# Veason-silverbullet/NNR

Hardware: NVIDIA B200
Metric: cne_sue_train_impressions_per_sec (higher is better)
Workload: dtype f32

## Files before the change

nnr_b200/csrc/gemm_tc.cu:

```cuda
#include "common.cuh"
#include "gemm_epilogue.cuh"
#include <cuda.h>
#include <cuda_bf16.h>
#include <stdlib.h>

extern "C" int nnr_gemm_default_algo(void);

#define TC_BM 128
#define TC_THREADS 320
#define TC_TMEM_COLS 512
#define TC_ACC_COLS 256
#define TC_EPI_PITCH 80
#define TC_EPI_SCRATCH (8 * 32 * TC_EPI_PITCH)
#define TC_SMEM_BUDGET (205 * 1024)
#define TC_CHAIN_K 2048

__device__ __forceinline__ uint32_t smem_u32(const void* p) { return (uint32_t)__cvta_generic_to_shared(p); }

__device__ __forceinline__ void mbar_init(uint64_t* bar, uint32_t count) {
  asm volatile("mbarrier.init.shared::cta.b64 [%0], %1;" ::"r"(smem_u32(bar)), "r"(count));
}
__device__ __forceinline__ void mbar_expect_tx(uint64_t* bar, uint32_t bytes) {
  asm volatile("mbarrier.arrive.expect_tx.shared::cta.b64 _, [%0], %1;" ::"r"(smem_u32(bar)), "r"(bytes) : "memory");
}
// ... 16 lines not shown
__device__ __forceinline__ void tma_load_3d(const CUtensorMap* map, uint64_t* bar, uint32_t dst, int c0, int c1, int c2) {
  asm volatile(
      "cp.async.bulk.tensor.3d.shared::cluster.global.mbarrier::complete_tx::bytes [%0], [%1, {%3, %4, %5}], [%2];"
      ::"r"(dst), "l"(map), "r"(smem_u32(bar)), "r"(c0), "r"(c1), "r"(c2)
      : "memory");
}
__device__ __forceinline__ void tc_fence_before() { asm volatile("tcgen05.fence::before_thread_sync;" ::: "memory"); }
__device__ __forceinline__ void tc_fence_after() { asm volatile("tcgen05.fence::after_thread_sync;" ::: "memory"); }
__device__ __forceinline__ void tc_commit(uint64_t* bar) {
  asm volatile("tcgen05.commit.cta_group::1.mbarrier::arrive::one.shared::cluster.b64 [%0];" ::"r"(smem_u32(bar)) : "memory");
}
template <bool BF16>
__device__ __forceinline__ void tc_mma(uint32_t d_tmem, uint64_t a_desc, uint64_t b_desc, uint32_t idesc, uint32_t accumulate) {
  if (BF16) {
    asm volatile(
        "{\n.reg .pred p;\nsetp.ne.b32 p, %4, 0;\n"
        "tcgen05.mma.cta_group::1.kind::f16 [%0], %1, %2, %3, p;\n}\n" ::"r"(d_tmem), "l"(a_desc), "l"(b_desc), "r"(idesc),
        "r"(accumulate)
        : "memory");
  } else {
    asm volatile(
        "{\n.reg .pred p;\nsetp.ne.b32 p, %4, 0;\n"
        "tcgen05.mma.cta_group::1.kind::tf32 [%0], %1, %2, %3, p;\n}\n" ::"r"(d_tmem), "l"(a_desc), "l"(b_desc), "r"(idesc),
        "r"(accumulate)
        : "memory");
  }
}
__device__ __forceinline__ uint32_t cluster_ctarank() {
  uint32_t r;
  asm volatile("mov.u32 %0, %%cluster_ctarank;" : "=r"(r));
  return r;
}
__device__ __forceinline__ uint32_t mapa_rank(uint32_t addr, uint32_t rank) {
  uint32_t r;
  asm volatile("mapa.shared::cluster.u32 %0, %1, %2;" : "=r"(r) : "r"(addr), "r"(rank));
  return r;
}
__device__ __forceinline__ void cluster_sync_all() {
  asm volatile("barrier.cluster.arrive.release.aligned;\nbarrier.cluster.wait.acquire.aligned;" ::: "memory");
}
__device__ __forceinline__ void tma_load_3d_pair(const CUtensorMap* map, uint32_t leader_bar, uint32_t dst, int c0, int c1, int c2) {
  asm volatile(
      "cp.async.bulk.tensor.3d.cta_group::2.shared::cluster.global.mbarrier::complete_tx::bytes [%0], [%1, {%3, %4, %5}], [%2];"
      ::"r"(dst), "l"(map), "r"(leader_bar), "r"(c0), "r"(c1), "r"(c2)
      : "memory");
}
__device__ __forceinline__ void tc_commit_pair(uint64_t* bar) {
  asm volatile("tcgen05.commit.cta_group::2.mbarrier::arrive::one.shared::cluster.multicast::cluster.b64 [%0], %1;" ::"r"(smem_u32(bar)),
               "h"((uint16_t)3)
               : "memory");
}
__device__ __forceinline__ void mbar_arrive_cluster(uint32_t cluster_addr) {
  asm volatile("mbarrier.arrive.release.cluster.shared::cluster.b64 _, [%0];" ::"r"(cluster_addr) : "memory");
}
template <bool BF16>
__device__ __forceinline__ void tc_mma_pair(uint32_t d_tmem, uint64_t a_desc, uint64_t b_desc, uint32_t idesc, uint32_t accumulate) {
  if (BF16) {
    asm volatile(
        "{\n.reg .pred p;\nsetp.ne.b32 p, %4, 0;\n"
        "tcgen05.mma.cta_group::2.kind::f16 [%0], %1, %2, %3, p;\n}\n" ::"r"(d_tmem), "l"(a_desc), "l"(b_desc), "r"(idesc),
        "r"(accumulate)
        : "memory");
  } else {
    asm volatile(
        "{\n.reg .pred p;\nsetp.ne.b32 p, %4, 0;\n"
        "tcgen05.mma.cta_group::2.kind::tf32 [%0], %1, %2, %3, p;\n}\n" ::"r"(d_tmem), "l"(a_desc), "l"(b_desc), "r"(idesc),
        "r"(accumulate)
        : "memory");
  }
}

__device__ __forceinline__ void tmem_ld16(uint32_t taddr, float* v) {
  uint32_t r[16];
  asm volatile(
      "tcgen05.ld.sync.aligned.32x32b.x16.b32 {%0, %1, %2, %3, %4, %5, %6, %7, %8, %9, %10, %11, %12, %13, %14, %15}, [%16];"
      : "=r"(r[0]), "=r"(r[1]), "=r"(r[2]), "=r"(r[3]), "=r"(r[4]), "=r"(r[5]), "=r"(r[6]), "=r"(r[7]), "=r"(r[8]), "=r"(r[9]),
        "=r"(r[10]), "=r"(r[11]), "=r"(r[12]), "=r"(r[13]), "=r"(r[14]), "=r"(r[15])
      : "r"(taddr));
  asm volatile("tcgen05.wait::ld.sync.aligned;" ::: "memory");
#pragma unroll
  for (int i = 0; i < 16; ++i) v[i] = __uint_as_float(r[i]);
}

__device__ __forceinline__ uint64_t make_sw128_desc(uint32_t smem_addr, uint32_t lbo_bytes, uint32_t sbo_bytes, uint32_t layout_type) {
  uint64_t d = 0;
  d |= (uint64_t)((smem_addr & 0x3FFFF) >> 4);
  d |= (uint64_t)((lbo_bytes >> 4) & 0x3FFF) << 16;
  d |= (uint64_t)((sbo_bytes >> 4) & 0x3FFF) << 32;
  d |= (uint64_t)1 << 46;
  d |= (uint64_t)layout_type << 61;
  return d;
}

#ifdef NNR_TC_PROF
__device__ unsigned long long g_tc_prof[16];
#define TC_STAMP(i) { if (blockIdx.x == 0) g_tc_prof[i] = clock64(); }
#else
#define TC_STAMP(i) {}
#endif

struct TcParams {
  int M, N, K;
  const int32_t* m_dev;
  const int32_t* k_dev;
  int block_n, stages, nplanes;
  int a_mn, b_mn;
// ... 178 lines not shown
            v.x *= ks[0]; v.y *= ks[1]; v.z *= ks[2]; v.w *= ks[3];
          }
        } else if (EP == NNR_EPI_GATE) {
          v.x = sigmoid_fast(v.x + rb[i].x); v.y = sigmoid_fast(v.y + rb[i].y);
          v.z = sigmoid_fast(v.z + rb[i].z); v.w = sigmoid_fast(v.w + rb[i].w);
          if (p.epi.aux_out) *reinterpret_cast<float4*>(p.epi.aux_out + t.o_ao[i] + n) = v;
          v.x *= ax[i].x; v.y *= ax[i].y; v.z *= ax[i].z; v.w *= ax[i].w;
        } else if (EP == NNR_EPI_ADD_AUX) {
          v.x += ax[i].x; v.y += ax[i].y; v.z += ax[i].z; v.w += ax[i].w;
        }
        if (acc_early) { v.x += ax[i].x; v.y += ax[i].y; v.z += ax[i].z; v.w += ax[i].w; }
        else if (accumulate) {
          const float4 cc = *reinterpret_cast<const float4*>(Cout + t.o_c[i] + n);
          v.x += cc.x; v.y += cc.y; v.z += cc.z; v.w += cc.w;
        }
        *reinterpret_cast<float4*>(Cout + t.o_c[i] + n) = v;
        if (planes) {
          const __nv_bfloat162 h01 = __floats2bfloat162_rn(v.x, v.y), h23 = __floats2bfloat162_rn(v.z, v.w);
          __nv_bfloat16* op = p.c_planes + (long long)(t.row0 + 8 * i) * p.c_pitch + n;
          uint2 hv;
          hv.x = *reinterpret_cast<const uint32_t*>(&h01); hv.y = *reinterpret_cast<const uint32_t*>(&h23);
          *reinterpret_cast<uint2*>(op) = hv;
          if (p.c_lo) {
            const __nv_bfloat162 l01 = __floats2bfloat162_rn(v.x - __low2float(h01), v.y - __high2float(h01));
            const __nv_bfloat162 l23 = __floats2bfloat162_rn(v.z - __low2float(h23), v.w - __high2float(h23));
            uint2 lv;
            lv.x = *reinterpret_cast<const uint32_t*>(&l01); lv.y = *reinterpret_cast<const uint32_t*>(&l23);
            *reinterpret_cast<uint2*>(op + p.c_pstride) = lv;
          }
        }
      }
      if (planes) {
        const int mz = min(p.c_rows, (M + 63) & ~63);
#pragma unroll
        for (int i = 0; i < 4; ++i) {
          const int mm = t.row0 + 8 * i;
          if (mm >= M && mm < mz) {
            __nv_bfloat16* op = p.c_planes + (long long)mm * p.c_pitch + n;
            *reinterpret_cast<uint2*>(op) = make_uint2(0u, 0u);
            if (p.c_lo) *reinterpret_cast<uint2*>(op + p.c_pstride) = make_uint2(0u, 0u);
          }
        }
      }
    }
    __syncwarp();
    if (AHEAD && more) {
      bb = bbn;
#pragma unroll
      for (int i = 0; i < 4; ++i) { ax[i] = axn[i]; rb[i] = rbn[i]; }
    }
  }
}

template <bool BF16, bool PAIR, int EPK>
__global__ void __launch_bounds__(TC_THREADS, 1) gemm_tc_kernel(const __grid_constant__ CUtensorMap map_a,
                                                                const __grid_constant__ CUtensorMap map_b, TcParams p) {
  extern __shared__ __align__(1024) unsigned char smem_raw[];
  constexpr int KELEM = BF16 ? 64 : 32;
  constexpr int TILE_M = PAIR ? 2 * TC_BM : TC_BM;
  int M = p.M, K = p.K;
  if (p.m_dev) M = min(M, *p.m_dev);
  if (p.k_dev) K = min(K, *p.k_dev);
  const int warp = threadIdx.x >> 5, lane = threadIdx.x & 31;
  if (threadIdx.x == 0) TC_STAMP(0)
  const uint32_t rank = PAIR ? cluster_ctarank() : 0u;
  const int sched_id = PAIR ? (int)(blockIdx.x >> 1) : (int)blockIdx.x;
  const int sched_n = PAIR ? (int)(gridDim.x >> 1) : (int)gridDim.x;
  const int b_rows = PAIR ? (p.block_n >> 1) : p.block_n;

  const int m_tiles = (M + TILE_M - 1) / TILE_M;
  const int n_tiles = (p.N + p.block_n - 1) / p.block_n;
  const int nkb = (K + KELEM - 1) / KELEM;
  const int kb_per = p.split_k ? p.chain_kb : max(nkb, 1);
  const int splits = p.split_k ? max(1, (nkb + kb_per - 1) / kb_per) : 1;
  const int total_tiles = m_tiles * n_tiles * splits;

  const uint32_t a_tile = TC_BM * 128, b_tile = (uint32_t)b_rows * 128;
  const uint32_t stage_bytes = (uint32_t)p.nplanes * (a_tile + b_tile);
  unsigned char* tiles = (unsigned char*)(((uintptr_t)smem_raw + 1023) & ~(uintptr_t)1023);
  unsigned char* epi_scratch = tiles + (size_t)p.stages * stage_bytes;
  uint64_t* full_bar = reinterpret_cast<uint64_t*>(epi_scratch + TC_EPI_SCRATCH);
  uint64_t* empty_bar = full_bar + p.stages;
  uint64_t* tmem_full = empty_bar + p.stages;
  uint64_t* tmem_empty = tmem_full + 2;
  uint32_t* tmem_slot = reinterpret_cast<uint32_t*>(tmem_empty + 2);

  if (warp == 0 && lane == 0) {
    asm volatile("prefetch.tensormap [%0];" ::"l"(&map_a) : "memory");
    asm volatile("prefetch.tensormap [%0];" ::"l"(&map_b) : "memory");
    for (int s = 0; s < p.stages; ++s) { mbar_init(&full_bar[s], 1); mbar_init(&empty_bar[s], 1); }
    for (int b = 0; b < 2; ++b) { mbar_init(&tmem_full[b], 1); mbar_init(&tmem_empty[b], PAIR ? 16 : 8); }
    asm volatile("fence.mbarrier_init.release.cluster;" ::: "memory");
  }
  if (PAIR) cluster_sync_all();
  if (warp == 1) {
    if (PAIR) {
      asm volatile("tcgen05.alloc.cta_group::2.sync.aligned.shared::cta.b32 [%0], %1;" ::"r"(smem_u32(tmem_slot)), "n"(TC_TMEM_COLS) : "memory");
      asm volatile("tcgen05.relinquish_alloc_permit.cta_group::2.sync.aligned;" ::: "memory");
    } else {
      asm volatile("tcgen05.alloc.cta_group::1.sync.aligned.shared::cta.b32 [%0], %1;" ::"r"(smem_u32(tmem_slot)), "n"(TC_TMEM_COLS) : "memory");
      asm volatile("tcgen05.relinquish_alloc_permit.cta_group::1.sync.aligned;" ::: "memory");
    }
  }
  tc_fence_before();
  __syncthreads();
  tc_fence_after();
  const uint32_t tmem_base = *tmem_slot;
  if (threadIdx.x == 0) TC_STAMP(1)

  if (warp == 0) {
    if (lane == 0) {
      int it = 0;
      for (int tile = sched_id; tile < total_tiles; tile += sched_n) {
        const int n_idx = tile % n_tiles, rest = tile / n_tiles;
        const int m0 = (rest % m_tiles) * TILE_M + (int)rank * TC_BM, n0 = n_idx * p.block_n + (int)rank * b_rows, z = rest / m_tiles;
        const int kb0 = z * kb_per, kb1 = min(nkb, kb0 + kb_per);
        for (int kb = kb0; kb < kb1; ++kb, ++it) {
          const int s = it % p.stages;
          const uint32_t ph = (it / p.stages) & 1;
          mbar_wait(&empty_bar[s], ph ^ 1);
          const uint32_t base = smem_u32(tiles + (size_t)s * stage_bytes);
          if (!PAIR) mbar_expect_tx(&full_bar[s], stage_bytes);
          else if (rank == 0) mbar_expect_tx(&full_bar[s], 2 * stage_bytes);
          const uint32_t lbar = PAIR ? mapa_rank(smem_u32(&full_bar[s]), 0) : 0u;
          auto load_a = [&](uint32_t dst, int c0, int c1, int c2) {
            if (PAIR) tma_load_3d_pair(&map_a, lbar, dst, c0, c1, c2); else tma_load_3d(&map_a, &full_bar[s], dst, c0, c1, c2);
          };
          auto load_b = [&](uint32_t dst, int c0, int c1, int c2) {
            if (PAIR) tma_load_3d_pair(&map_b, lbar, dst, c0, c1, c2); else tma_load_3d(&map_b, &full_bar[s], dst, c0, c1, c2);
          };
          for (int pl = 0; pl < p.nplanes; ++pl) {
            const uint32_t sa = base + pl * a_tile;
            const uint32_t sb = base + p.nplanes * a_tile + pl * b_tile;
            if (!p.a_mn) load_a(sa, kb * KELEM, m0, pl);
            else for (int g = 0; g < TC_BM / KELEM; ++g) load_a(sa + g * (KELEM * 128), m0 + g * KELEM, kb * KELEM, pl);
            if (!p.b_mn) load_b(sb, kb * KELEM, n0, pl);
            else for (int g = 0; g < b_rows / KELEM; ++g) load_b(sb + g * (KELEM * 128), n0 + g * KELEM, kb * KELEM, pl);
          }
        }
      }
    }
  } else if (warp == 1) {
    if (lane == 0 && rank == 0) {
      int it = 0, tl = 0;
      const uint32_t lbo = KELEM * 128;
      const uint64_t a_step = p.a_mn ? (uint64_t)((BF16 ? 2048 : 1024) >> 4) : 2;
      const uint64_t b_step = p.b_mn ? (uint64_t)((BF16 ? 2048 : 1024) >> 4) : 2;
      for (int tile = sched_id; tile < total_tiles; tile += sched_n, ++tl) {
        const int rest = tile / n_tiles;
        const int z = rest / m_tiles;
        const int kb0 = z * kb_per, kb1 = min(nkb, kb0 + kb_per);
        const int buf = tl & 1;
        mbar_wait(&tmem_empty[buf], ((tl >> 1) & 1) ^ 1);
        tc_fence_after();
        const uint32_t d_tmem = tmem_base + buf * TC_ACC_COLS;
        uint32_t first = 1;
        for (int kb = kb0; kb < kb1; ++kb, ++it) {
          const int s = it % p.stages;
          mbar_wait(&full_bar[s], (it / p.stages) & 1);
          tc_fence_after();
          if (it == 0) TC_STAMP(2)
          const uint32_t base = smem_u32(tiles + (size_t)s * stage_bytes);
          const uint32_t a_lt = (p.a_mn && !BF16) ? 1u : 2u, a_sbo = (p.a_mn && !BF16) ? 512u : 1024u;
          const uint32_t b_lt = (p.b_mn && !BF16) ? 1u : 2u, b_sbo = (p.b_mn && !BF16) ? 512u : 1024u;
          const uint64_t a_hi = make_sw128_desc(base, p.a_mn ? lbo : 0, a_sbo, a_lt);
          const uint64_t a_lo = make_sw128_desc(base + a_tile, p.a_mn ? lbo : 0, a_sbo, a_lt);
          const uint64_t b_hi = make_sw128_desc(base + p.nplanes * a_tile, p.b_mn ? lbo : 0, b_sbo, b_lt);
          const uint64_t b_lo = make_sw128_desc(base + p.nplanes * a_tile + b_tile, p.b_mn ? lbo : 0, b_sbo, b_lt);
#pragma unroll
          for (int k = 0; k < 4; ++k) {
            const uint64_t ao = a_step * k, bo = b_step * k;
            if (PAIR) tc_mma_pair<BF16>(d_tmem, a_hi + ao, b_hi + bo, p.idesc, first ? 0u : 1u);
            else tc_mma<BF16>(d_tmem, a_hi + ao, b_hi + bo, p.idesc, first ? 0u : 1u);
            first = 0;
            if (p.nplanes == 2) {
              if (PAIR) {
                tc_mma_pair<BF16>(d_tmem, a_hi + ao, b_lo + bo, p.idesc, 1u);
                tc_mma_pair<BF16>(d_tmem, a_lo + ao, b_hi + bo, p.idesc, 1u);
              } else {
                tc_mma<BF16>(d_tmem, a_hi + ao, b_lo + bo, p.idesc, 1u);
                tc_mma<BF16>(d_tmem, a_lo + ao, b_hi + bo, p.idesc, 1u);
              }
            }
          }
          if (PAIR) tc_commit_pair(&empty_bar[s]); else tc_commit(&empty_bar[s]);
        }
        if (tl < 2) TC_STAMP(3 + tl)
        if (PAIR) tc_commit_pair(&tmem_full[buf]); else tc_commit(&tmem_full[buf]);
      }
    }
  } else {
    const int q = warp & 3;
    const int chalf = (warp - 2) >> 2;
    const uint64_t drop_seed = (p.epi.p_drop > 0.f) ? nnr_resolve_seed(p.epi.seed) : 0ull;
    const int nchunks = p.block_n >> 4;
    const int c_begin = chalf ? ((nchunks + 1) >> 1) << 4 : 0;
    const int c_end = chalf ? p.block_n : ((nchunks + 1) >> 1) << 4;
    int tl = 0;
    for (int tile = sched_id; tile < total_tiles; tile += sched_n, ++tl) {
      const int n_idx = tile % n_tiles, rest = tile / n_tiles;
      const int m0 = (rest % m_tiles) * TILE_M + (int)rank * TC_BM, n0 = n_idx * p.block_n, z = rest / m_tiles;
      const int kb0 = z * kb_per, kb1 = min(nkb, kb0 + kb_per);
      const int buf = tl & 1;
      const uint32_t lane_addr = tmem_base + buf * TC_ACC_COLS + ((uint32_t)(q * 32) << 16);
      unsigned char* my_tile = epi_scratch + (size_t)(warp - 2) * 32 * TC_EPI_PITCH;
      const int tr = lane >> 2, tc4 = (lane & 3) * 4;
      int rmap[4] = {0, 0, 0, 0};
      if ((EPK < 0 || EPK == NNR_EPI_GATE) && p.epi.epilogue == NNR_EPI_GATE && !p.partial) {
#pragma unroll
        for (int i = 0; i < 4; ++i) {
          const int mm = m0 + q * 32 + tr + 8 * i;
          if (mm < M) rmap[i] = __ldg(p.epi.rowmap + mm);
        }
      }
      const bool fast = EPK >= 0;
      uint32_t o_c[4], o_aux[4], o_ao[4], o_rb[4];
      uint32_t rvalid = 0;
      if (fast) {
#pragma unroll
        for (int i = 0; i < 4; ++i) {
          const int mm = m0 + q * 32 + tr + 8 * i;
          if (mm < M) rvalid |= 1u << i;
          const uint32_t mr = (mm < M) ? (uint32_t)mm : 0u;
          o_c[i] = (EPK == TC_EPK_PARTIAL) ? ((uint32_t)z * (uint32_t)M + mr) * (uint32_t)p.N : mr * (uint32_t)p.epi.ldc;
          o_aux[i] = mr * (uint32_t)p.epi.ldaux;
          o_ao[i] = mr * (uint32_t)p.epi.ldaux_out;
          o_rb[i] = (uint32_t)rmap[i] * (uint32_t)p.epi.ldrowbias;
        }
      }
      mbar_wait(&tmem_full[buf], (tl >> 1) & 1);
      tc_fence_after();
      if (warp == 2 && lane == 0 && tl < 2) TC_STAMP(5 + 2 * tl)
      if (EPK >= 0) {
        EpiTile et;
#pragma unroll
        for (int i = 0; i < 4; ++i) { et.o_c[i] = o_c[i]; et.o_aux[i] = o_aux[i]; et.o_ao[i] = o_ao[i]; et.o_rb[i] = o_rb[i]; }
        et.rvalid = rvalid; et.row0 = m0 + q * 32 + tr;
        epi_tile_fast<(EPK >= 0 ? EPK : 0)>(p, et, lane_addr, kb1 > kb0, c_begin, c_end, n0, smem_u32(my_tile), lane, M, drop_seed,
// ... 6 lines not shown
#pragma unroll
          for (int i = 0; i < 16; ++i) v[i] = 0.f;
        }
#pragma unroll
        for (int qd = 0; qd < 4; ++qd)
          *reinterpret_cast<float4*>(my_tile + lane * TC_EPI_PITCH + qd * 16) = make_float4(v[4 * qd], v[4 * qd + 1], v[4 * qd + 2], v[4 * qd + 3]);
        __syncwarp();
        const int n = n0 + c0 + tc4;
        const int cnt = min(4, p.N - n);
        float o[4][4];
#pragma unroll
        for (int i = 0; i < 4; ++i) {
          const float4 x = *reinterpret_cast<const float4*>(my_tile + (tr + 8 * i) * TC_EPI_PITCH + tc4 * 4);
          o[i][0] = x.x; o[i][1] = x.y; o[i][2] = x.z; o[i][3] = x.w;
        }
        if (cnt > 0) {
          if (p.partial) {
#pragma unroll
            for (int i = 0; i < 4; ++i) {
              const int mm = m0 + q * 32 + tr + 8 * i;
              if (mm < M) st4(p.partial + ((size_t)z * M + mm) * p.N + n, cnt, o[i]);
            }
          } else {
            Epi4In in[4];
            float bias4[4] = {0.f, 0.f, 0.f, 0.f};
            if (p.epi.bias && (p.epi.epilogue == NNR_EPI_BIAS || p.epi.epilogue == NNR_EPI_BIAS_TANH || p.epi.epilogue == NNR_EPI_BIAS_RELU_RES))
              ld4(p.epi.bias + n, cnt, bias4);
#pragma unroll
            for (int i = 0; i < 4; ++i) {
              const int mm = m0 + q * 32 + tr + 8 * i;
              if (mm < M) epi_load4(p.epi, mm, n, cnt, in[i], rmap[i]);
            }
#pragma unroll
            for (int i = 0; i < 4; ++i) {
              const int mm = m0 + q * 32 + tr + 8 * i;
              if (mm < M) epi_finish4(p.epi, mm, n, o[i], cnt, bias4, in[i]);
            }
          }
        }
        __syncwarp();
      }
      tc_fence_before();
      __syncwarp();
      if (warp == 2 && lane == 0 && tl < 2) TC_STAMP(6 + 2 * tl)
      if (lane == 0) {
        if (PAIR && rank != 0) mbar_arrive_cluster(mapa_rank(smem_u32(&tmem_empty[buf]), 0));
        else mbar_arrive(&tmem_empty[buf]);
      }
    }
  }
  tc_fence_before();
  __syncthreads();
  if (threadIdx.x == 0) TC_STAMP(9)
  if (PAIR) cluster_sync_all();
  if (warp == 1) {
    if (PAIR) asm volatile("tcgen05.dealloc.cta_group::2.sync.aligned.b32 %0, %1;" ::"r"(tmem_base), "n"(TC_TMEM_COLS) : "memory");
    else asm volatile("tcgen05.dealloc.cta_group::1.sync.aligned.b32 %0, %1;" ::"r"(tmem_base), "n"(TC_TMEM_COLS) : "memory");
  }
}

__global__ void tc_splitk_reduce_kernel(const float* __restrict__ partial, int K, const int32_t* __restrict__ k_dev, int kelem,
                                        int chain_kb, int M, int N, const int32_t* __restrict__ m_dev, EpiP epi) {
  if (m_dev) M = min(M, *m_dev);
  if (k_dev) K = min(K, *k_dev);
  const int nkb = (K + kelem - 1) / kelem;
  const int splits = max(1, (nkb + chain_kb - 1) / chain_kb);
  size_t i = (size_t)blockIdx.x * blockDim.x + threadIdx.x;
  if (i >= (size_t)M * N) return;
  int m = (int)(i / N), n = (int)(i - (size_t)m * N);
  float acc = 0.f;
  for (int s = 0; s < splits; ++s) acc += partial[((size_t)s * M + m) * N + n];
  epi_store(epi, m, n, acc);
}
__global__ void __launch_bounds__(256) tc_splitk_reduce4_kernel(const float* __restrict__ partial, int K, const int32_t* __restrict__ k_dev,
                                                                int kelem, int chain_kb, int M, int N, const int32_t* __restrict__ m_dev,
                                                                EpiP epi) {
  if (m_dev) M = min(M, *m_dev);
  if (k_dev) K = min(K, *k_dev);
  const int nkb = (K + kelem - 1) / kelem;
  const int splits = max(1, (nkb + chain_kb - 1) / chain_kb);
  const int N4 = N >> 2;
  const size_t i = (size_t)blockIdx.x * blockDim.x + threadIdx.x;
  if (i >= (size_t)M * N4) return;
  const int m = (int)(i / N4), n = (int)(i - (size_t)m * N4) * 4;
  const size_t plane = (size_t)M * N;
  const float* src = partial + (size_t)m * N + n;
  float4 acc = make_float4(0.f, 0.f, 0.f, 0.f);
  int s = 0;
  for (; s + 4 <= splits; s += 4) {
    float4 v[4];
#pragma unroll
    for (int u = 0; u < 4; ++u) v[u] = __ldg(reinterpret_cast<const float4*>(src + (size_t)(s + u) * plane));
#pragma unroll
    for (int u = 0; u < 4; ++u) { acc.x += v[u].x; acc.y += v[u].y; acc.z += v[u].z; acc.w += v[u].w; }
  }
  for (; s < splits; ++s) {
    const float4 v = __ldg(reinterpret_cast<const float4*>(src + (size_t)s * plane));
    acc.x += v.x; acc.y += v.y; acc.z += v.z; acc.w += v.w;
  }
  float o[4] = {acc.x, acc.y, acc.z, acc.w};
  float bias4[4] = {0.f, 0.f, 0.f, 0.f};
  if (epi.bias && (epi.epilogue == NNR_EPI_BIAS || epi.epilogue == NNR_EPI_BIAS_TANH || epi.epilogue == NNR_EPI_BIAS_RELU_RES))
    ld4(epi.bias + n, 4, bias4);
  Epi4In in;
  epi_load4(epi, m, n, 4, in, epi.epilogue == NNR_EPI_GATE ? __ldg(epi.rowmap + m) : 0);
  epi_finish4(epi, m, n, o, 4, bias4, in);
}
// ... 177 lines not shown
    }
  }
}
__global__ void __launch_bounds__(512) tc_split_colsum_reduce(const float* __restrict__ partial, int nblocks, int R, int C, int Cp,
                                                              const int32_t* __restrict__ r_dev, float* __restrict__ out, int accumulate) {
  __shared__ float s_sum[16][33];
  const int cl = threadIdx.x & 31, sl = threadIdx.x >> 5;
  const int c = blockIdx.x * 32 + cl;
  int Rv = R;
  if (r_dev) Rv = min(R, *r_dev);
  const int nb = min(nblocks, (Rv + tcs_rows(R) - 1) / tcs_rows(R));
  float a0 = 0.f, a1 = 0.f;
  if (c < C) {
    int b = sl;
    for (; b + 16 < nb; b += 32) { a0 += partial[(size_t)b * Cp + c]; a1 += partial[(size_t)(b + 16) * Cp + c]; }
    if (b < nb) a0 += partial[(size_t)b * Cp + c];
  }
  s_sum[sl][cl] = a0 + a1;
  __syncthreads();
  if (sl == 0 && c < C) {
    float acc = 0.f;
#pragma unroll
    for (int q = 0; q < 16; ++q) acc += s_sum[q][cl];
    out[c] = accumulate ? out[c] + acc : acc;
  }
}

typedef CUresult (*EncodeTiledFn)(CUtensorMap*, CUtensorMapDataType, cuuint32_t, void*, const cuuint64_t*, const cuuint64_t*,
                                  const cuuint32_t*, const cuuint32_t*, CUtensorMapInterleave, CUtensorMapSwizzle,
                                  CUtensorMapL2promotion, CUtensorMapFloatOOBfill);
static EncodeTiledFn get_encode() {
  static EncodeTiledFn fn = nullptr;
  static bool tried = false;
  if (!tried) {
    tried = true;
    void* p = nullptr;
    cudaDriverEntryPointQueryResult q;
    if (cudaGetDriverEntryPoint("cuTensorMapEncodeTiled", &p, cudaEnableDefault, &q) == cudaSuccess && q == cudaDriverEntryPointSuccess)
      fn = (EncodeTiledFn)p;
    else (void)cudaGetLastError();
  }
  return fn;
}

static size_t up(size_t x, size_t a) { return (x + a - 1) / a * a; }

struct TcPlan {
  bool bf16;
  int a_mn, b_mn;
  int a_rows, a_cols, b_rows, b_cols;
  int a_cp, b_cp;
  int block_n, stages, split_k, chain_kb, max_splits, nplanes, kelem;
  int pair;
  size_t a_plane, b_plane, a_off, b_off, partial_off, total, smem;
};

static double stage_penalty() {
  static double v = -1.0;
  if (v < 0) { const char* e = getenv("NNR_TC_STAGE_PENALTY"); v = e ? atof(e) : 1.3; }
  return v;
}
static double stage_penalty3() {
  static double v = -1.0;
  if (v < 0) { const char* e = getenv("NNR_TC_STAGE_PENALTY3"); v = e ? atof(e) : 1.0; }
  return v;
}
static int pick_block_n(int N, int step, int nplanes) {
  int best = step;
  double best_cost = 1e30;
  for (int bn = 256; bn >= 32; bn -= step) {
    double padded = (double)((N + bn - 1) / bn) * bn;
    double cost = padded * (1.0 + 40.0 / bn);
    size_t stage = (size_t)nplanes * ((size_t)TC_BM * 128 + (size_t)bn * 128);
    if (TC_SMEM_BUDGET / stage < 3) cost *= stage_penalty();
    else if (TC_SMEM_BUDGET / stage < 4) cost *= stage_penalty3();
    if (cost < best_cost - 1e-9) { best_cost = cost; best = bn; }
  }
  return best;
}

static int chain_k_limit() {
  static int v = -1;
  if (v < 0) { const char* e = getenv("NNR_TC_CHAIN_K"); v = e ? atoi(e) : TC_CHAIN_K; if (v < 256) v = 256; }
  return v;
}
static int fast_epilogue_enabled() {
  static int v = -1;
  if (v < 0) { const char* e = getenv("NNR_TC_FAST_EPILOGUE"); v = e ? atoi(e) : 1; }
  return v;
}
static int pair_mode() {
  static int v = -1;
  if (v < 0) { const char* e = getenv("NNR_TC_PAIR"); v = e ? atoi(e) : 1; }
  return v;
}
static int pair_min_m() {
  static int v = -1;
  if (v < 0) { const char* e = getenv("NNR_TC_PAIR_MIN_M"); v = e ? atoi(e) : 2 * TC_BM * 148; }
  return v;
}
static int pair_min_tiles() {
  static int v = -1;
  if (v < 0) { const char* e = getenv("NNR_TC_PAIR_MIN_TILES"); v = e ? atoi(e) : 48; }
  return v;
}
static int pick_block_n_pair(int N, int step, int nplanes) {
  int best = 0;
  double best_cost = 1e30;
  for (int bn = 256; bn >= 64; bn -= step) {
    size_t stage = (size_t)nplanes * ((size_t)TC_BM * 128 + (size_t)(bn / 2) * 128);
    if (TC_SMEM_BUDGET / stage < 3) continue;
    double padded = (double)((N + bn - 1) / bn) * bn;
    if (padded > 1.15 * N) continue;
    double cost = padded * (1.0 + 40.0 / bn);
    if (cost < best_cost - 1e-9) { best_cost = cost; best = bn; }
  }
  return best;
}

static int algo_mode(int algo) {
  if (algo == NNR_GEMM_AUTO) algo = nnr_gemm_default_algo();
  return algo == NNR_GEMM_TC_BF16 ? 1 : (algo == NNR_GEMM_TC_BF16X3 ? 2 : 0);
}
static TcPlan make_plan(const nnr_gemm_args* a, int mode) {
  TcPlan pl;
  const bool bf16 = mode != 0;
  pl.bf16 = bf16;
  pl.kelem = bf16 ? 64 : 32;
  pl.nplanes = mode == 1 ? 1 : 2;
  pl.a_mn = a->transA ? 1 : 0;
  pl.b_mn = a->transB ? 0 : 1;
  pl.a_rows = a->transA ? a->K : a->M; pl.a_cols = a->transA ? a->M : a->K;
  pl.b_rows = a->transB ? a->N : a->K; pl.b_cols = a->transB ? a->K : a->N;
  const size_t pad = bf16 ? 8 : 4;
  pl.a_cp = (int)up((size_t)pl.a_cols, pad);
  pl.b_cp = (int)up((size_t)pl.b_cols, pad);
  pl.block_n = pick_block_n(a->N, pl.b_mn ? pl.kelem : 16, pl.nplanes);
  pl.pair = 0;
  if (pair_mode() && a->M >= pair_min_m() && !(a->transA) && a->k_dev == nullptr) {
    int bnp = pick_block_n_pair(a->N, pl.b_mn ? 2 * pl.kelem : 16, pl.nplanes);
    if (bnp && a->M < 2 * TC_BM * 148) {
      long ptiles = (long)((a->M + 2 * TC_BM - 1) / (2 * TC_BM)) * ((a->N + bnp - 1) / bnp);
      if (ptiles < pair_min_tiles()) bnp = 0;
    }
    if (bnp) { pl.pair = 1; pl.block_n = bnp; }
  }
  long tiles = (long)((a->M + TC_BM - 1) / TC_BM) * ((a->N + pl.block_n - 1) / pl.block_n);
  int nkb_cap = (a->K + pl.kelem - 1) / pl.kelem;
  pl.split_k = 0;
  const int chain_k = chain_k_limit();
  pl.chain_kb = chain_k / pl.kelem;
  if (!pl.pair && tiles * 2 <= 148 && nkb_cap >= 8) {
    int target = (int)((148 + tiles - 1) / tiles);
    int chain = (nkb_cap + target - 1) / target;
    if (chain < 4) chain = 4;
    if (chain > chain_k / pl.kelem) chain = chain_k / pl.kelem;
    if (chain < nkb_cap) { pl.split_k = 1; pl.chain_kb = chain; }
  }
  pl.max_splits = pl.split_k ? (nkb_cap + pl.chain_kb - 1) / pl.chain_kb : 1;
  size_t stage = (size_t)pl.nplanes * ((size_t)TC_BM * 128 + (size_t)(pl.pair ? pl.block_n / 2 : pl.block_n) * 128);
  int stages = (int)(TC_SMEM_BUDGET / stage);
  if (stages < 2) stages = 2;
  if (stages > 6) stages = 6;
  pl.stages = stages;
  pl.smem = 1024 + (size_t)stages * stage + TC_EPI_SCRATCH + (2 * stages + 4) * 8 + 16;
  const size_t esz = bf16 ? 2 : 4;
  pl.a_plane = (size_t)pl.a_rows * pl.a_cp;
  pl.b_plane = (size_t)pl.b_rows * pl.b_cp;
  size_t o = 0;
  pl.a_off = o; if (!a->A_planes) o = up(o + pl.a_plane * esz * pl.nplanes, 1024);
  pl.b_off = o; if (!a->B_planes) o = up(o + pl.b_plane * esz * pl.nplanes, 1024);
  pl.partial_off = o;
  if (pl.split_k) o = up(o + (size_t)pl.max_splits * a->M * a->N * sizeof(float), 1024);
  pl.total = o;
  return pl;
}

int nnr_gemm_tc_supported(const nnr_gemm_args* a) {
  static int disabled = -1;
  if (disabled < 0) { const char* e = getenv("NNR_DISABLE_TC"); disabled = (e && e[0] == '1') ? 1 : 0; }
  if (disabled) return 0;
  if (!get_encode()) return 0;
  if ((double)a->M * a->N * a->K < 2.0e6 && a->A && a->B) return 0;
  if (a->K < 8) return 0;
  if (a->m_dev && a->transA) return 0;
  if (a->k_dev && !(a->transA && !a->transB)) return 0;
  return 1;
}

size_t nnr_gemm_tc_workspace_bytes(const nnr_gemm_args* a) { return make_plan(a, algo_mode(a->algo)).total; }

static int encode_map(CUtensorMap* map, const void* base, bool bf16, int cols, int64_t pitch, int rows, int64_t plane_rows,
                      int nplanes, int box_c, int box_r, bool mn) {
  cuuint64_t gdim[3] = {(cuuint64_t)cols, (cuuint64_t)rows, (cuuint64_t)nplanes};
  const size_t esz = bf16 ? 2 : 4;
  cuuint64_t gstr[2] = {(cuuint64_t)pitch * esz, (cuuint64_t)pitch * esz * (cuuint64_t)plane_rows};
  cuuint32_t box[3] = {(cuuint32_t)box_c, (cuuint32_t)box_r, 1};
  cuuint32_t estr[3] = {1, 1, 1};
  CUresult r = get_encode()(map, bf16 ? CU_TENSOR_MAP_DATA_TYPE_BFLOAT16 : CU_TENSOR_MAP_DATA_TYPE_FLOAT32, 3, const_cast<void*>(base), gdim, gstr,
                            box, estr, CU_TENSOR_MAP_INTERLEAVE_NONE,
                            (mn && !bf16) ? CU_TENSOR_MAP_SWIZZLE_128B_ATOM_32B : CU_TENSOR_MAP_SWIZZLE_128B,
                            CU_TENSOR_MAP_L2_PROMOTION_L2_256B, CU_TENSOR_MAP_FLOAT_OOB_FILL_NONE);
  if (r != CUDA_SUCCESS) { nnr_set_error("nnr_gemm(tc): cuTensorMapEncodeTiled failed (%d)", (int)r); return NNR_ERR_ARG; }
  return 0;
}

template <int MODE>
static int split_operand(const float* X, int64_t ld, int R, int C, int Cp, const int32_t* r_dev, void* out, size_t plane_stride,
                         cudaStream_t st) {
  bool vec = nnr_aligned16(X) && (ld % 4 == 0);
  long long total = (long long)R * (Cp / 4);
  long long want = (total + 256 * 4 - 1) / (256 * 4);
  int grid = (int)(want < 148 * 16 ? want : 148 * 16);
  if (grid < 1) grid = 1;
  void* ph = nnr_prof_begin(1, 0.0, st);
  tc_split_kernel<MODE><<<grid, 256, 0, st>>>(X, ld, R, C, Cp, r_dev, vec, out, plane_stride);
  nnr_prof_end(ph, st);
  NNR_LAUNCH_CHECK("tc_split_kernel");
  return 0;
}

template <bool BF16, bool PAIR>
static const void* tc_kernel_ptr2(int epk) {
  if (!BF16) return (const void*)gemm_tc_kernel<BF16, PAIR, -1>;
  switch (epk) {
    case NNR_EPI_NONE: return (const void*)gemm_tc_kernel<BF16, PAIR, BF16 ? NNR_EPI_NONE : -1>;
    case NNR_EPI_BIAS: return (const void*)gemm_tc_kernel<BF16, PAIR, BF16 ? NNR_EPI_BIAS : -1>;
    case NNR_EPI_BIAS_TANH: return (const void*)gemm_tc_kernel<BF16, PAIR, BF16 ? NNR_EPI_BIAS_TANH : -1>;
    case NNR_EPI_BIAS_RELU_RES: return (const void*)gemm_tc_kernel<BF16, PAIR, BF16 ? NNR_EPI_BIAS_RELU_RES : -1>;
    case NNR_EPI_GATE: return (const void*)gemm_tc_kernel<BF16, PAIR, BF16 ? NNR_EPI_GATE : -1>;
    case NNR_EPI_ADD_AUX: return (const void*)gemm_tc_kernel<BF16, PAIR, BF16 ? NNR_EPI_ADD_AUX : -1>;
    case TC_EPK_PARTIAL: return (const void*)gemm_tc_kernel<BF16, PAIR, BF16 ? TC_EPK_PARTIAL : -1>;
    default: return (const void*)gemm_tc_kernel<BF16, PAIR, -1>;
  }
}
template <bool BF16>
static const void* tc_kernel_ptr(bool pair, int epk) {
  return pair ? tc_kernel_ptr2<BF16, true>(epk) : tc_kernel_ptr2<BF16, false>(epk);
}

template <int MODE>
static int run_tc(const nnr_gemm_args* a, cudaStream_t st) {
  constexpr bool BF16 = MODE != 0;
  TcPlan pl = make_plan(a, MODE);
  NNR_REQUIRE(pl.total == 0 || (a->workspace && a->workspace_bytes >= pl.total), NNR_ERR_WORKSPACE,
              "nnr_gemm(tc): workspace %zu < %zu", a->workspace_bytes, pl.total);
  NNR_REQUIRE(nnr_aligned16(a->workspace), NNR_ERR_ALIGN, "nnr_gemm(tc): workspace must be 16B aligned");
  NNR_REQUIRE(nnr_aligned16(a->A_planes) && nnr_aligned16(a->B_planes) && a->a_planes_pitch % (BF16 ? 8 : 4) == 0 &&
                  a->b_planes_pitch % (BF16 ? 8 : 4) == 0,
              NNR_ERR_ALIGN, "nnr_gemm(tc): operand planes must be 16B aligned with a 16B pitch");
  NNR_REQUIRE(pl.smem <= 227 * 1024, NNR_ERR_UNSUPPORTED, "nnr_gemm(tc): smem plan too large");
  char* ws = (char*)a->workspace;
  const void* pa = a->A_planes;
  const void* pb = a->B_planes;
  int64_t a_pitch = a->a_planes_pitch, a_prow = a->a_planes_rows, b_pitch = a->b_planes_pitch, b_prow = a->b_planes_rows;
  int rc;
  if (!pa) {
    void* w = ws + pl.a_off;
    rc = split_operand<MODE>(a->A, a->lda, pl.a_rows, pl.a_cols, pl.a_cp, pl.a_mn ? a->k_dev : a->m_dev, w, pl.a_plane, st);
    if (rc) return rc;
    pa = w; a_pitch = pl.a_cp; a_prow = pl.a_rows;
  }
  if (!pb) {
    void* w = ws + pl.b_off;
    rc = split_operand<MODE>(a->B, a->ldb, pl.b_rows, pl.b_cols, pl.b_cp, pl.b_mn ? a->k_dev : nullptr, w, pl.b_plane, st);
    if (rc) return rc;
    pb = w; b_pitch = pl.b_cp; b_prow = pl.b_rows;
  }
  CUtensorMap map_a, map_b;
  const int ke = pl.kelem;
  rc = encode_map(&map_a, pa, BF16, pl.a_cols, a_pitch, pl.a_rows, a_prow, pl.nplanes, ke, pl.a_mn ? ke : TC_BM, pl.a_mn != 0);
  if (rc) return rc;
  rc = encode_map(&map_b, pb, BF16, pl.b_cols, b_pitch, pl.b_rows, b_prow, pl.nplanes, ke,
                  pl.b_mn ? ke : (pl.pair ? pl.block_n / 2 : pl.block_n), pl.b_mn != 0);
  if (rc) return rc;
  TcParams p;
  p.M = a->M; p.N = a->N; p.K = a->K; p.m_dev = a->m_dev; p.k_dev = a->k_dev;
  p.block_n = pl.block_n; p.stages = pl.stages; p.nplanes = pl.nplanes;
  p.a_mn = pl.a_mn; p.b_mn = pl.b_mn; p.split_k = pl.split_k; p.chain_kb = pl.chain_kb;
  const uint32_t fmt = BF16 ? 1u : 2u;
  p.idesc = (1u << 4) | (fmt << 7) | (fmt << 10) | ((uint32_t)pl.a_mn << 15) | ((uint32_t)pl.b_mn << 16) |
            ((uint32_t)(pl.block_n >> 3) << 17) | ((uint32_t)((pl.pair ? 2 * TC_BM : TC_BM) >> 4) << 24);
  p.partial = pl.split_k ? (float*)(ws + pl.partial_off) : nullptr;
  p.epi = make_epi(a);
  {
    auto ok = [](const void* ptr, int64_t ld) { return !ptr || (nnr_aligned16(ptr) && ld % 4 == 0); };
    p.epi_fast = (a->N % 4 == 0) && ok(a->C, a->ldc) && ok(a->aux, a->ldaux) && ok(a->aux_out, a->ldaux_out) &&
                 ok(a->rowbias, a->ldrowbias) && ok(a->bias, 4) && fast_epilogue_enabled();
    if (a->epilogue == NNR_EPI_GATE && !(a->rowbias && a->rowmap && a->aux)) p.epi_fast = 0;
    if (a->epilogue == NNR_EPI_ADD_AUX && !a->aux) p.epi_fast = 0;
    const double lim = 4294967296.0;
    if ((double)a->M * (double)a->ldc >= lim || (double)a->M * (double)a->ldaux >= lim || (double)a->M * (double)a->ldaux_out >= lim ||
        (double)a->M * (double)a->ldrowbias >= lim)
      p.epi_fast = 0;
  }
  p.c_planes = nullptr; p.c_pitch = 0; p.c_pstride = 0; p.c_lo = 0; p.c_rows = 0;
  if (a->C_planes) {
    NNR_REQUIRE(BF16 && p.epi_fast && !pl.split_k && a->N % 8 == 0 && a->c_planes_pitch >= a->N && a->c_planes_pitch % 8 == 0 &&
                    a->c_planes_rows >= a->M && nnr_aligned16(a->C_planes),
                NNR_ERR_UNSUPPORTED, "nnr_gemm: C_planes needs a bf16 tensor-core algo, N %% 8 == 0, aligned epilogue operands, no split-K");
    p.c_planes = (__nv_bfloat16*)a->C_planes;
    p.c_pitch = a->c_planes_pitch;
    p.c_pstride = a->c_planes_rows * a->c_planes_pitch;
    p.c_lo = pl.nplanes == 2;
    p.c_rows = (int)a->c_planes_rows;
  }
  static bool attr_set[16][2][2][8] = {};
  static int num_sms_tab[16] = {};
  int dev = 0;
  NNR_CUDA(cudaGetDevice(&dev));
  dev &= 15;
  int epk = (BF16 && p.epi_fast && !pl.split_k) ? a->epilogue : -1;
  if (BF16 && pl.split_k && fast_epilogue_enabled() && a->N % 4 == 0 && nnr_aligned16(p.partial) &&
      (double)pl.max_splits * (double)a->M * (double)a->N < 4294967296.0)
    epk = TC_EPK_PARTIAL;
  const void* kernel = tc_kernel_ptr<BF16>(pl.pair != 0, epk);
  if (!attr_set[dev][BF16 ? 1 : 0][pl.pair][epk + 1]) {
    NNR_CUDA(cudaFuncSetAttribute(kernel, cudaFuncAttributeMaxDynamicSharedMemorySize, 227 * 1024));
    attr_set[dev][BF16 ? 1 : 0][pl.pair][epk + 1] = true;
  }
  if (num_sms_tab[dev] == 0) NNR_CUDA(cudaDeviceGetAttribute(&num_sms_tab[dev], cudaDevAttrMultiProcessorCount, dev));
  const int num_sms = num_sms_tab[dev];
  void* ph = nnr_prof_begin(0, -1.0, st);
  {
    cudaLaunchConfig_t cfg = {};
    cudaLaunchAttribute attr[1];
    if (pl.pair) {
      long cap_tiles = (long)((a->M + 2 * TC_BM - 1) / (2 * TC_BM)) * ((a->N + pl.block_n - 1) / pl.block_n);
      long pairs = cap_tiles < num_sms / 2 ? cap_tiles : num_sms / 2;
      attr[0].id = cudaLaunchAttributeClusterDimension;
      attr[0].val.clusterDim.x = 2; attr[0].val.clusterDim.y = 1; attr[0].val.clusterDim.z = 1;
      cfg.attrs = attr; cfg.numAttrs = 1;
      cfg.gridDim = dim3((unsigned)(2 * pairs));
    } else {
      long cap_tiles = (long)((a->M + TC_BM - 1) / TC_BM) * ((a->N + pl.block_n - 1) / pl.block_n) * pl.max_splits;
      cfg.gridDim = dim3((unsigned)(cap_tiles < num_sms ? cap_tiles : num_sms));
    }
    cfg.blockDim = dim3(TC_THREADS); cfg.dynamicSmemBytes = pl.smem; cfg.stream = st;
    void* kargs[] = {(void*)&map_a, (void*)&map_b, (void*)&p};
    cudaError_t e = cudaLaunchKernelExC(&cfg, kernel, kargs);
    nnr_count_launch(1);
    if (e != cudaSuccess) { nnr_set_error("gemm_tc_kernel(%s): launch failed: %s", pl.pair ? "pair" : "single", cudaGetErrorString(e)); return (int)e; }
    nnr_prof_end(ph, st);
  }
  if (pl.split_k) {
    size_t tot = (size_t)a->M * a->N;
    void* ph2 = nnr_prof_begin(2, 0.0, st);
    if (a->N % 4 == 0 && nnr_aligned16(p.partial))
      tc_splitk_reduce4_kernel<<<(unsigned)((tot / 4 + 255) / 256), 256, 0, st>>>(p.partial, a->K, a->k_dev, pl.kelem, pl.chain_kb, a->M,
                                                                                 a->N, a->m_dev, p.epi);
    else
      tc_splitk_reduce_kernel<<<(unsigned)((tot + 255) / 256), 256, 0, st>>>(p.partial, a->K, a->k_dev, pl.kelem, pl.chain_kb, a->M,
                                                                            a->N, a->m_dev, p.epi);
    nnr_prof_end(ph2, st);
    NNR_LAUNCH_CHECK("tc_splitk_reduce_kernel");
  }
  return 0;
}

int nnr_gemm_tc(const nnr_gemm_args* a, void* stream) {
  cudaStream_t st = (cudaStream_t)stream;
  const int mode = algo_mode(a->algo);
  if (mode == 1) return run_tc<1>(a, st);
  if (mode == 2) return run_tc<2>(a, st);
  return run_tc<0>(a, st);
}

extern "C" int64_t nnr_tc_split_pitch(int C, int algo) { return (int64_t)up((size_t)C, algo_mode(algo) ? 8 : 4); }
extern "C" size_t nnr_tc_split_bytes(int R, int C, int algo) {
  if (R <= 0 || C <= 0) return 0;
  const int mode = algo_mode(algo);
  return (size_t)R * (size_t)nnr_tc_split_pitch(C, algo) * (mode == 0 ? 8 : (mode == 1 ? 2 : 4));
}
extern "C" int nnr_tc_split(const float* X, int64_t ld, int R, int C, const int32_t* r_dev, int algo, void* planes,
                            size_t planes_bytes, void* stream) {
  NNR_REQUIRE(X && planes && R > 0 && C > 0 && ld >= C, NNR_ERR_ARG, "nnr_tc_split: bad arguments");
  NNR_REQUIRE(planes_bytes >= nnr_tc_split_bytes(R, C, algo), NNR_ERR_WORKSPACE, "nnr_tc_split: planes buffer too small");
  NNR_REQUIRE(nnr_aligned16(planes), NNR_ERR_ALIGN, "nnr_tc_split: planes must be 16B aligned");
  const int mode = algo_mode(algo);
  int Cp = (int)nnr_tc_split_pitch(C, algo);
  if (mode == 1) return split_operand<1>(X, ld, R, C, Cp, r_dev, planes, (size_t)R * Cp, (cudaStream_t)stream);
  if (mode == 2) return split_operand<2>(X, ld, R, C, Cp, r_dev, planes, (size_t)R * Cp, (cudaStream_t)stream);
  return split_operand<0>(X, ld, R, C, Cp, r_dev, planes, (size_t)R * Cp, (cudaStream_t)stream);
}

extern "C" size_t nnr_tc_split_colsum_workspace_bytes(int R, int C, int algo) {
  if (R <= 0 || C <= 0) return 0;
  return (size_t)((R + tcs_rows(R) - 1) / tcs_rows(R)) * (size_t)nnr_tc_split_pitch(C, algo) * sizeof(float);
}
extern "C" int nnr_tc_split_colsum(const float* X, int64_t ld, int R, int C, const int32_t* r_dev, int algo, void* planes,
                                   size_t planes_bytes, float* colsum, int accumulate, void* workspace, size_t workspace_bytes,
                                   void* stream) {
  NNR_REQUIRE(X && planes && colsum && workspace && R > 0 && C > 0 && ld >= C, NNR_ERR_ARG, "nnr_tc_split_colsum: bad arguments");
  NNR_REQUIRE(planes_bytes >= nnr_tc_split_bytes(R, C, algo), NNR_ERR_WORKSPACE, "nnr_tc_split_colsum: planes buffer too small");
  NNR_REQUIRE(workspace_bytes >= nnr_tc_split_colsum_workspace_bytes(R, C, algo), NNR_ERR_WORKSPACE,
// ... 273 lines not shown
```

Measured before the change: 9678.

## Add cluster TMA multicast of A tiles for split-K tensor-core GEMM

Adds a clustered kernel variant for non-pair split-K GEMMs with a partial-sum epilogue. CTAs in a cluster of 2-4 share the A operand through TMA multicast: each CTA issues a subset of the A boxes to all cluster members, and MMA commits signal every CTA's empty barrier. The aim is to cut redundant global/L2 reads of A across the N tiles. In exchange it adds cross-CTA barrier coupling, a drain wait at the end of the producer loop, and an occupancy query to size the cluster grid. The scheduler assumes cluster members hold the same M and split index and differ only in N tile.

```diff
diff --git a/nnr_b200/csrc/gemm_tc.cu b/nnr_b200/csrc/gemm_tc.cu
--- a/nnr_b200/csrc/gemm_tc.cu
+++ b/nnr_b200/csrc/gemm_tc.cu
@@ -92,6 +92,22 @@
 }
 __device__ __forceinline__ void mbar_arrive_cluster(uint32_t cluster_addr) {
   asm volatile("mbarrier.arrive.release.cluster.shared::cluster.b64 _, [%0];" ::"r"(cluster_addr) : "memory");
+}
+__device__ __forceinline__ uint32_t cluster_nctarank() {
+  uint32_t r;
+  asm volatile("mov.u32 %0, %%cluster_nctarank;" : "=r"(r));
+  return r;
+}
+__device__ __forceinline__ void tma_load_3d_mc(const CUtensorMap* map, uint64_t* bar, uint32_t dst, int c0, int c1, int c2, uint16_t mask) {
+  asm volatile(
+      "cp.async.bulk.tensor.3d.shared::cluster.global.mbarrier::complete_tx::bytes.multicast::cluster [%0], [%1, {%3, %4, %5}], [%2], %6;"
+      ::"r"(dst), "l"(map), "r"(smem_u32(bar)), "r"(c0), "r"(c1), "r"(c2), "h"(mask)
+      : "memory");
+}
+__device__ __forceinline__ void tc_commit_mc(uint64_t* bar, uint16_t mask) {
+  asm volatile("tcgen05.commit.cta_group::1.mbarrier::arrive::one.shared::cluster.multicast::cluster.b64 [%0], %1;" ::"r"(smem_u32(bar)),
+               "h"(mask)
+               : "memory");
 }
 template <bool BF16>
 __device__ __forceinline__ void tc_mma_pair(uint32_t d_tmem, uint64_t a_desc, uint64_t b_desc, uint32_t idesc, uint32_t accumulate) {
@@ -376,7 +392,7 @@
   }
 }
 
-template <bool BF16, bool PAIR, int EPK>
+template <bool BF16, bool PAIR, int EPK, bool MC>
 __global__ void __launch_bounds__(TC_THREADS, 1) gemm_tc_kernel(const __grid_constant__ CUtensorMap map_a,
                                                                 const __grid_constant__ CUtensorMap map_b, TcParams p) {
   extern __shared__ __align__(1024) unsigned char smem_raw[];
@@ -388,6 +404,9 @@
   const int warp = threadIdx.x >> 5, lane = threadIdx.x & 31;
   if (threadIdx.x == 0) TC_STAMP(0)
   const uint32_t rank = PAIR ? cluster_ctarank() : 0u;
+  const uint32_t mc_rank = MC ? cluster_ctarank() : 0u;
+  const uint32_t csize = MC ? cluster_nctarank() : 1u;
+  const uint16_t mc_mask = (uint16_t)((1u << csize) - 1u);
   const int sched_id = PAIR ? (int)(blockIdx.x >> 1) : (int)blockIdx.x;
   const int sched_n = PAIR ? (int)(gridDim.x >> 1) : (int)gridDim.x;
   const int b_rows = PAIR ? (p.block_n >> 1) : p.block_n;
@@ -412,11 +431,11 @@
   if (warp == 0 && lane == 0) {
     asm volatile("prefetch.tensormap [%0];" ::"l"(&map_a) : "memory");
     asm volatile("prefetch.tensormap [%0];" ::"l"(&map_b) : "memory");
-    for (int s = 0; s < p.stages; ++s) { mbar_init(&full_bar[s], 1); mbar_init(&empty_bar[s], 1); }
+    for (int s = 0; s < p.stages; ++s) { mbar_init(&full_bar[s], 1); mbar_init(&empty_bar[s], csize); }
     for (int b = 0; b < 2; ++b) { mbar_init(&tmem_full[b], 1); mbar_init(&tmem_empty[b], PAIR ? 16 : 8); }
     asm volatile("fence.mbarrier_init.release.cluster;" ::: "memory");
   }
-  if (PAIR) cluster_sync_all();
+  if (PAIR || MC) cluster_sync_all();
   if (warp == 1) {
     if (PAIR) {
       asm volatile("tcgen05.alloc.cta_group::2.sync.aligned.shared::cta.b32 [%0], %1;" ::"r"(smem_u32(tmem_slot)), "n"(TC_TMEM_COLS) : "memory");
@@ -447,8 +466,11 @@
           if (!PAIR) mbar_expect_tx(&full_bar[s], stage_bytes);
           else if (rank == 0) mbar_expect_tx(&full_bar[s], 2 * stage_bytes);
           const uint32_t lbar = PAIR ? mapa_rank(smem_u32(&full_bar[s]), 0) : 0u;
+          int a_box = 0;
           auto load_a = [&](uint32_t dst, int c0, int c1, int c2) {
-            if (PAIR) tma_load_3d_pair(&map_a, lbar, dst, c0, c1, c2); else tma_load_3d(&map_a, &full_bar[s], dst, c0, c1, c2);
+            if (PAIR) tma_load_3d_pair(&map_a, lbar, dst, c0, c1, c2);
+            else if (MC) { if ((uint32_t)(a_box++) % csize == mc_rank) tma_load_3d_mc(&map_a, &full_bar[s], dst, c0, c1, c2, mc_mask); }
+            else tma_load_3d(&map_a, &full_bar[s], dst, c0, c1, c2);
           };
           auto load_b = [&](uint32_t dst, int c0, int c1, int c2) {
             if (PAIR) tma_load_3d_pair(&map_b, lbar, dst, c0, c1, c2); else tma_load_3d(&map_b, &full_bar[s], dst, c0, c1, c2);
@@ -463,6 +485,8 @@
           }
         }
       }
+      if (MC)
+        for (int j = max(0, it - p.stages); j < it; ++j) mbar_wait(&empty_bar[j % p.stages], (j / p.stages) & 1);
     }
   } else if (warp == 1) {
     if (lane == 0 && rank == 0) {
@@ -507,7 +531,7 @@
               }
             }
           }
-          if (PAIR) tc_commit_pair(&empty_bar[s]); else tc_commit(&empty_bar[s]);
+          if (PAIR) tc_commit_pair(&empty_bar[s]); else if (MC) tc_commit_mc(&empty_bar[s], mc_mask); else tc_commit(&empty_bar[s]);
         }
         if (tl < 2) TC_STAMP(3 + tl)
         if (PAIR) tc_commit_pair(&tmem_full[buf]); else tc_commit(&tmem_full[buf]);
@@ -620,7 +644,7 @@
   tc_fence_before();
   __syncthreads();
   if (threadIdx.x == 0) TC_STAMP(9)
-  if (PAIR) cluster_sync_all();
+  if (PAIR || MC) cluster_sync_all();
   if (warp == 1) {
     if (PAIR) asm volatile("tcgen05.dealloc.cta_group::2.sync.aligned.b32 %0, %1;" ::"r"(tmem_base), "n"(TC_TMEM_COLS) : "memory");
     else asm volatile("tcgen05.dealloc.cta_group::1.sync.aligned.b32 %0, %1;" ::"r"(tmem_base), "n"(TC_TMEM_COLS) : "memory");
@@ -904,6 +928,7 @@
   int a_cp, b_cp;
   int block_n, stages, split_k, chain_kb, max_splits, nplanes, kelem;
   int pair;
+  int cluster;
   size_t a_plane, b_plane, a_off, b_off, partial_off, total, smem;
 };
 
@@ -1010,6 +1035,12 @@
     if (chain < nkb_cap) { pl.split_k = 1; pl.chain_kb = chain; }
   }
   pl.max_splits = pl.split_k ? (nkb_cap + pl.chain_kb - 1) / pl.chain_kb : 1;
+  pl.cluster = 1;
+  if (pl.split_k && !pl.pair && mode == 2) {
+    const int n_tiles = (a->N + pl.block_n - 1) / pl.block_n;
+    for (int c = 4; c >= 2; --c)
+      if (n_tiles % c == 0) { pl.cluster = c; break; }
+  }
   size_t stage = (size_t)pl.nplanes * ((size_t)TC_BM * 128 + (size_t)(pl.pair ? pl.block_n / 2 : pl.block_n) * 128);
   int stages = (int)(TC_SMEM_BUDGET / stage);
   if (stages < 2) stages = 2;
@@ -1074,21 +1105,24 @@
 
 template <bool BF16, bool PAIR>
 static const void* tc_kernel_ptr2(int epk) {
-  if (!BF16) return (const void*)gemm_tc_kernel<BF16, PAIR, -1>;
+  if (!BF16) return (const void*)gemm_tc_kernel<BF16, PAIR, -1, false>;
   switch (epk) {
-    case NNR_EPI_NONE: return (const void*)gemm_tc_kernel<BF16, PAIR, BF16 ? NNR_EPI_NONE : -1>;
-    case NNR_EPI_BIAS: return (const void*)gemm_tc_kernel<BF16, PAIR, BF16 ? NNR_EPI_BIAS : -1>;
-    case NNR_EPI_BIAS_TANH: return (const void*)gemm_tc_kernel<BF16, PAIR, BF16 ? NNR_EPI_BIAS_TANH : -1>;
-    case NNR_EPI_BIAS_RELU_RES: return (const void*)gemm_tc_kernel<BF16, PAIR, BF16 ? NNR_EPI_BIAS_RELU_RES : -1>;
-    case NNR_EPI_GATE: return (const void*)gemm_tc_kernel<BF16, PAIR, BF16 ? NNR_EPI_GATE : -1>;
-    case NNR_EPI_ADD_AUX: return (const void*)gemm_tc_kernel<BF16, PAIR, BF16 ? NNR_EPI_ADD_AUX : -1>;
-    case TC_EPK_PARTIAL: return (const void*)gemm_tc_kernel<BF16, PAIR, BF16 ? TC_EPK_PARTIAL : -1>;
-    default: return (const void*)gemm_tc_kernel<BF16, PAIR, -1>;
+    case NNR_EPI_NONE: return (const void*)gemm_tc_kernel<BF16, PAIR, BF16 ? NNR_EPI_NONE : -1, false>;
+    case NNR_EPI_BIAS: return (const void*)gemm_tc_kernel<BF16, PAIR, BF16 ? NNR_EPI_BIAS : -1, false>;
+    case NNR_EPI_BIAS_TANH: return (const void*)gemm_tc_kernel<BF16, PAIR, BF16 ? NNR_EPI_BIAS_TANH : -1, false>;
+    case NNR_EPI_BIAS_RELU_RES: return (const void*)gemm_tc_kernel<BF16, PAIR, BF16 ? NNR_EPI_BIAS_RELU_RES : -1, false>;
+    case NNR_EPI_GATE: return (const void*)gemm_tc_kernel<BF16, PAIR, BF16 ? NNR_EPI_GATE : -1, false>;
+    case NNR_EPI_ADD_AUX: return (const void*)gemm_tc_kernel<BF16, PAIR, BF16 ? NNR_EPI_ADD_AUX : -1, false>;
+    case TC_EPK_PARTIAL: return (const void*)gemm_tc_kernel<BF16, PAIR, BF16 ? TC_EPK_PARTIAL : -1, false>;
+    default: return (const void*)gemm_tc_kernel<BF16, PAIR, -1, false>;
   }
 }
 template <bool BF16>
-static const void* tc_kernel_ptr(bool pair, int epk) {
-  return pair ? tc_kernel_ptr2<BF16, true>(epk) : tc_kernel_ptr2<BF16, false>(epk);
+static const void* tc_kernel_ptr(int variant, int epk) {
+  if constexpr (BF16) {
+    if (variant == 2) return (const void*)gemm_tc_kernel<true, false, TC_EPK_PARTIAL, true>;
+  }
+  return variant == 1 ? tc_kernel_ptr2<BF16, true>(epk) : tc_kernel_ptr2<BF16, false>(epk);
 }
 
 template <int MODE>
@@ -1157,8 +1191,10 @@
     p.c_lo = pl.nplanes == 2;
     p.c_rows = (int)a->c_planes_rows;
   }
-  static bool attr_set[16][2][2][8] = {};
+  static bool attr_set[16][2][3][8] = {};
   static int num_sms_tab[16] = {};
+  static int mc_clusters_tab[16][5] = {};
+  static size_t mc_smem_tab[16][5] = {};
   int dev = 0;
   NNR_CUDA(cudaGetDevice(&dev));
   dev &= 15;
@@ -1166,10 +1202,12 @@
   if (BF16 && pl.split_k && fast_epilogue_enabled() && a->N % 4 == 0 && nnr_aligned16(p.partial) &&
       (double)pl.max_splits * (double)a->M * (double)a->N < 4294967296.0)
     epk = TC_EPK_PARTIAL;
-  const void* kernel = tc_kernel_ptr<BF16>(pl.pair != 0, epk);
-  if (!attr_set[dev][BF16 ? 1 : 0][pl.pair][epk + 1]) {
+  const int mc = (pl.cluster > 1 && epk == TC_EPK_PARTIAL) ? pl.cluster : 1;
+  const int variant = pl.pair ? 1 : (mc > 1 ? 2 : 0);
+  const void* kernel = tc_kernel_ptr<BF16>(variant, epk);
+  if (!attr_set[dev][BF16 ? 1 : 0][variant][epk + 1]) {
     NNR_CUDA(cudaFuncSetAttribute(kernel, cudaFuncAttributeMaxDynamicSharedMemorySize, 227 * 1024));
-    attr_set[dev][BF16 ? 1 : 0][pl.pair][epk + 1] = true;
+    attr_set[dev][BF16 ? 1 : 0][variant][epk + 1] = true;
   }
   if (num_sms_tab[dev] == 0) NNR_CUDA(cudaDeviceGetAttribute(&num_sms_tab[dev], cudaDevAttrMultiProcessorCount, dev));
   const int num_sms = num_sms_tab[dev];
@@ -1177,6 +1215,7 @@
   {
     cudaLaunchConfig_t cfg = {};
     cudaLaunchAttribute attr[1];
+    cfg.blockDim = dim3(TC_THREADS); cfg.dynamicSmemBytes = pl.smem; cfg.stream = st;
     if (pl.pair) {
       long cap_tiles = (long)((a->M + 2 * TC_BM - 1) / (2 * TC_BM)) * ((a->N + pl.block_n - 1) / pl.block_n);
       long pairs = cap_tiles < num_sms / 2 ? cap_tiles : num_sms / 2;
@@ -1184,15 +1223,28 @@
       attr[0].val.clusterDim.x = 2; attr[0].val.clusterDim.y = 1; attr[0].val.clusterDim.z = 1;
       cfg.attrs = attr; cfg.numAttrs = 1;
       cfg.gridDim = dim3((unsigned)(2 * pairs));
+    } else if (mc > 1) {
+      long cap_units = (long)((a->M + TC_BM - 1) / TC_BM) * ((a->N + pl.block_n - 1) / pl.block_n) / mc * pl.max_splits;
+      attr[0].id = cudaLaunchAttributeClusterDimension;
+      attr[0].val.clusterDim.x = mc; attr[0].val.clusterDim.y = 1; attr[0].val.clusterDim.z = 1;
+      cfg.attrs = attr; cfg.numAttrs = 1;
+      if (mc_smem_tab[dev][mc] != pl.smem) {
+        cfg.gridDim = dim3((unsigned)(mc * (num_sms / mc)));
+        NNR_CUDA(cudaOccupancyMaxActiveClusters(&mc_clusters_tab[dev][mc], kernel, &cfg));
+        NNR_REQUIRE(mc_clusters_tab[dev][mc] > 0, NNR_ERR_UNSUPPORTED, "nnr_gemm(tc): no cluster of %d CTAs fits (%zu B shared memory)", mc,
+                    pl.smem);
+        mc_smem_tab[dev][mc] = pl.smem;
+      }
+      long clusters = cap_units < mc_clusters_tab[dev][mc] ? cap_units : mc_clusters_tab[dev][mc];
+      cfg.gridDim = dim3((unsigned)(mc * clusters));
     } else {
       long cap_tiles = (long)((a->M + TC_BM - 1) / TC_BM) * ((a->N + pl.block_n - 1) / pl.block_n) * pl.max_splits;
       cfg.gridDim = dim3((unsigned)(cap_tiles < num_sms ? cap_tiles : num_sms));
     }
-    cfg.blockDim = dim3(TC_THREADS); cfg.dynamicSmemBytes = pl.smem; cfg.stream = st;
     void* kargs[] = {(void*)&map_a, (void*)&map_b, (void*)&p};
     cudaError_t e = cudaLaunchKernelExC(&cfg, kernel, kargs);
     nnr_count_launch(1);
-    if (e != cudaSuccess) { nnr_set_error("gemm_tc_kernel(%s): launch failed: %s", pl.pair ? "pair" : "single", cudaGetErrorString(e)); return (int)e; }
+    if (e != cudaSuccess) { nnr_set_error("gemm_tc_kernel(%s): launch failed: %s", pl.pair ? "pair" : (mc > 1 ? "multicast" : "single"), cudaGetErrorString(e)); return (int)e; }
     nnr_prof_end(ph, st);
   }
   if (pl.split_k) {
```

Result: slower. 9327 (median of 6 runs) (-3.6%).
